# tobifinn/torch-assimilate

Hardware: AMD Instinct MI355X
Metric: local analyses/sec (LETKF, 40-member) (higher is better)
Workload: dtype f32

## Files before the change

### include/mia_letkf.h

```cpp
#ifndef MIA_LETKF_H
#define MIA_LETKF_H

#include <stddef.h>
#include <stdint.h>

#ifdef __cplusplus
extern "C" {
#endif

#define MIA_VERSION 100

#define MIA_OK 0
#define MIA_ERR_NULL (-1)
#define MIA_ERR_SIZE (-2)
#define MIA_ERR_UNSUPPORTED (-3)
#define MIA_ERR_WORKSPACE (-4)
#define MIA_ERR_ALIGN (-5)
#define MIA_ERR_COMM (-6)
#define MIA_ERR_ARG (-7)

#define MIA_FLAG_OVERFLOW 1
#define MIA_FLAG_NOCONV 2
#define MIA_FLAG_NONFINITE 4
#define MIA_FLAG_RETRY 8
// ... 98 lines not shown
                                 int32_t* flags, int32_t* retry_count, void* stream);
int mia_letkf_weights_retry_f32(const float* X, int64_t ldx, int m, int k, int64_t g0, int64_t g1,
                                const float* rec, int64_t P,
                                const int32_t* nbr_cnt, const int32_t* nbr_idx, const double* nbr_w,
                                int p_cap, int p_max, float inf_factor, float gamma,
                                float* Xa, int64_t ldo, int64_t o0, float* W, int32_t* flags, void* stream);
#define MIA_TILE_BOX_OVERFLOW (1 << 30)
#define MIA_STEP_STATUS_SAMPLED 64
#define MIA_STEP_STATUS_NONFINITE 128
int mia_letkf_tile_lists_bytes(int64_t n_points, int p_max, int extra_blocks, size_t* bytes);
int mia_letkf_localize_tiles_f64(int taper, const double* grid_xyz, int64_t g0, int64_t g1,
                                 const double* obs_xyz, int64_t P, int n_coord,
                                 const int32_t* coord_group , const double* gc_c , int n_r,
                                 double gc_eps, int p_max, int extra_blocks, void* tile_lists, size_t tile_lists_bytes,
                                 int32_t* stats, void* ws, size_t ws_bytes, void* stream);
int mia_letkf_localize_tiles_periodic_f64(int taper, const double* grid_xyz, int64_t g0, int64_t g1,
                                          const double* obs_xyz, int64_t P, int n_coord,
                                          const int32_t* coord_group , const double* period ,
                                          const double* gc_c , int n_r, double gc_eps, int p_max, int extra_blocks, void* tile_lists, size_t tile_lists_bytes,
                                          int32_t* stats, void* ws, size_t ws_bytes, void* stream);
int mia_letkf_split_record_bytes(int k, size_t* bytes);
int mia_letkf_pack_split_f32(const float* Yb, const float* d, int k, int64_t P, void* split_rec ,
                             void* stream);
int mia_letkf_analysis_tiles_f32(const float* X, int64_t ldx, int m, int k, int64_t g0, int64_t g1,
                                 const void* split_rec, int64_t P, const void* tile_lists, int p_max, int extra_blocks,
                                 float inf_factor, float* Xa, int64_t ldo, int64_t o0, int32_t* flags,
                                 int32_t* retry_count, void* stream);
int mia_letkf_weights_tiles_f32(const float* X, int64_t ldx, int m, int k, int64_t g0, int64_t g1,
                                const void* split_rec, int64_t P, const void* tile_lists, int p_max, int extra_blocks,
                                float inf_factor, float* Xa, int64_t ldo, int64_t o0, float* W ,
                                int32_t* flags, int32_t* retry_count, void* stream);

int mia_letkf_tiles_cover(int m, int k, int p_max, int extra_blocks, int64_t ldx, int64_t ldo, int64_t n_points, int64_t P,
                          float gamma);
int mia_lketkf_rbf_analysis_tiles_f32(const float* X, int64_t ldx, int m, int k, int64_t g0, int64_t g1,
                                      const float* Yb, const float* d, int64_t P, const void* tile_lists, int p_max,
                                      int extra_blocks, float inf_factor, float gamma, float* Xa, int64_t ldo, int64_t o0,
                                      int32_t* flags, int32_t* retry_count, void* stream);

int mia_letkf_analysis_matfun_fused_f32(const float* X, int64_t ldx, int m, int k, int64_t g0, int64_t g1,
                                        const float* rec, int64_t P,
                                        const double* grid_xyz, int n_coord, const int32_t* coord_group ,
                                        const double* gc_c , int n_r, double gc_eps,
                                        void* index_ws, size_t index_ws_bytes,
                                        int p_max_assumed, float inf_factor, float gamma,
                                        float* Xa, int64_t ldo, int64_t o0, int32_t* flags, int32_t* retry_count,
// ... 274 lines not shown
```

### torch-assimilate_amd/_cabi.py

```python
import ctypes as C
import os

from ._build import LIB_PATH

_lib = None

i32, i64, f32, f64, vp, sz = C.c_int, C.c_int64, C.c_float, C.c_double, C.c_void_p, C.c_size_t


class KernelOp(C.Structure):
    _fields_ = [("op", C.c_int32), ("reserved", C.c_int32), ("value", C.c_double)]


_PROTOS = {
    "mia_version": ([], i32),
    "mia_status_string": ([i32], C.c_char_p),
    "mia_set_option": ([C.c_char_p, i32], i32),
    "mia_get_option": ([C.c_char_p, C.POINTER(C.c_int)], i32),
    "mia_last_analysis_kernel": ([C.c_char_p, i32], i32),
    "mia_last_transform_kernel": ([C.c_char_p, i32], i32),
    "mia_gaspari_cohn_f64": ([vp, i64, vp, vp], i32),
    "mia_gaspari_cohn_f32": ([vp, i64, vp, vp], i32),
    "mia_gaspari_cohn_inf_f64": ([vp, i64, vp, vp], i32),
    "mia_gaspari_cohn_inf_f32": ([vp, i64, vp, vp], i32),
# ... 45 lines not shown
                                      vp, i64, i64, vp, vp, vp, vp], i32),
    "mia_letkf_weights_retry_f64": ([vp, i64, i32, i32, i64, i64, vp, i64, vp, vp, vp, i32, i32, f64, f64,
                                     vp, i64, i64, vp, vp, vp], i32),
    "mia_letkf_weights_f64_cover": ([i32, i32, i64, i64], i32),
    "mia_letkf_weights_matfun_f32": ([vp, i64, i32, i32, i64, i64, vp, i64, vp, vp, vp, i32, i32, f32, f32,
                                      vp, i64, i64, vp, vp, vp, vp], i32),
    "mia_letkf_weights_retry_f32": ([vp, i64, i32, i32, i64, i64, vp, i64, vp, vp, vp, i32, i32, f32, f32,
                                     vp, i64, i64, vp, vp, vp], i32),
    "mia_letkf_index_build_f64": ([vp, i64, i32, C.POINTER(C.c_int32), C.POINTER(f64), i32, vp, sz, vp], i32),
    "mia_letkf_index_build_periodic_f64": ([vp, i64, i32, C.POINTER(C.c_int32), C.POINTER(f64), C.POINTER(f64), i32, vp, sz, vp],
                                           i32),
    "mia_letkf_localize_taper_periodic_f64": ([i32, vp, i64, i64, vp, i64, i32, C.POINTER(C.c_int32), C.POINTER(f64),
                                               C.POINTER(f64), i32, f64, i32, vp, vp, vp, vp, vp, sz, vp], i32),
    "mia_letkf_localize_tiles_periodic_f64": ([i32, vp, i64, i64, vp, i64, i32, C.POINTER(C.c_int32), C.POINTER(f64),
                                               C.POINTER(f64), i32, f64, i32, i32, vp, sz, vp, vp, sz, vp], i32),
    "mia_letkf_analysis_matfun_fused_f32": ([vp, i64, i32, i32, i64, i64, vp, i64, vp, i32, C.POINTER(C.c_int32),
                                             C.POINTER(f64), i32, f64, vp, sz, i32, f32, f32, vp, i64, i64, vp, vp, vp,
                                             vp], i32),
    "mia_letkf_tile_lists_bytes": ([i64, i32, i32, C.POINTER(sz)], i32),
    "mia_letkf_localize_tiles_f64": ([i32, vp, i64, i64, vp, i64, i32, C.POINTER(C.c_int32), C.POINTER(f64), i32, f64,
                                      i32, i32, vp, sz, vp, vp, sz, vp], i32),
    "mia_letkf_split_record_bytes": ([i32, C.POINTER(sz)], i32),
    "mia_letkf_pack_split_f32": ([vp, vp, i32, i64, vp, vp], i32),
    "mia_letkf_analysis_tiles_f32": ([vp, i64, i32, i32, i64, i64, vp, i64, vp, i32, i32, f32, vp, i64, i64, vp, vp, vp], i32),
    "mia_letkf_tiles_cover": ([i32, i32, i32, i32, i64, i64, i64, i64, f32], i32),
    "mia_lketkf_rbf_analysis_tiles_f32": ([vp, i64, i32, i32, i64, i64, vp, vp, i64, vp, i32, i32, f32, f32, vp, i64, i64,
                                           vp, vp, vp], i32),
    "mia_letkf_weights_tiles_f32": ([vp, i64, i32, i32, i64, i64, vp, i64, vp, i32, i32, f32, vp, i64, i64, vp, vp, vp, vp], i32),
    "mia_letkf_analysis_retry_f32": ([vp, i64, i32, i32, i64, i64, vp, i64, vp, vp, vp, i32, i32, f32, f32,
                                      vp, i64, i64, vp, vp], i32),
    "mia_lketkf_rbf_analysis_f32": ([vp, i64, i32, i32, i64, i64, vp, vp, i64, vp, vp, vp, i32, i32, f32, f32,
                                     vp, i64, i64, vp, vp, vp, sz, vp], i32),
    "mia_lketkf_rbf_analysis_f64": ([vp, i64, i32, i32, i64, i64, vp, vp, i64, vp, vp, vp, i32, i32, f64, f64,
                                     vp, i64, i64, vp, vp, vp, sz, vp], i32),
    "mia_etkf_workspace_bytes": ([i32, i64, i32, C.POINTER(sz)], i32),
    "mia_etkf_weights_f32": ([vp, vp, i32, i64, f32, vp, vp, vp, sz, vp], i32),
    "mia_etkf_weights_f64": ([vp, vp, i32, i64, f64, vp, vp, vp, sz, vp], i32),
    "mia_ketkf_workspace_bytes": ([i32, i64, i32, C.POINTER(sz)], i32),
    "mia_ketkf_weights_f32": ([vp, vp, i32, i64, f32, C.POINTER(KernelOp), i32, vp, vp, vp, sz, vp], i32),
    "mia_ketkf_weights_f64": ([vp, vp, i32, i64, f64, C.POINTER(KernelOp), i32, vp, vp, vp, sz, vp], i32),
    "mia_apply_weights_f32": ([vp, i64, i32, i32, i64, i64, vp, vp, i64, i64, vp], i32),
    "mia_apply_weights_f64": ([vp, i64, i32, i32, i64, i64, vp, vp, i64, i64, vp], i32),
    "mia_apply_f64_cover": ([i32, i32, i64, i64, i64], i32),
    "mia_apply_local_f64_cover": ([i32, i32, i64, i64, i64], i32),
    "mia_apply_local_weights_f32": ([vp, i64, i32, i32, i64, i64, vp, vp, i64, i64, vp], i32),
    "mia_apply_local_weights_f64": ([vp, i64, i32, i32, i64, i64, vp, vp, i64, i64, vp], i32),
# ... 153 lines not shown
```

### torch-assimilate_amd/csrc/localize.hip

```cpp
#include <cstdlib>
#include "mia_common.h"
#include "mia_options.h"
#include "mia_localize_dev.h"
#include "mia_pack_dev.h"
#include "mia_tiles.h"

namespace mia {


struct IndexParams {
  const double* obs;
  int64_t P;
  int nc;
  double cutoff[MIA_MAX_COORD];
  int cell_cap;
  IndexHeader* hdr;
  int* start;
  int* cursor;
  int* sorted;
  int* cell_of;
  int* rank_of;
  double* sxyz;
  unsigned nb_bbox;
  PackJob pack;
// ... 530 lines not shown
  unsigned nb_pack = 0;
  if (pack && pack->rec) {
    if ((P + 63) / 64 > 2000000000LL) return MIA_ERR_UNSUPPORTED;
    ip.pack = *pack;
    nb_pack = (unsigned)((P + 63) / 64);
  }
  const size_t pack_lds = nb_pack ? (size_t)64 * (ip.pack.kp + 1) * sizeof(float) : 0;
  index_bbox_dims_kernel<<<dim3(ip.nb_bbox + nb_pack), dim3(kPrepThreads), pack_lds, stream>>>(ip);
  MIA_LAUNCH_CHECK();
  count_k<<<dim3(nbP), dim3(kPrepThreads), 0, stream>>>(ip);
  MIA_LAUNCH_CHECK();
  index_scan_kernel<<<dim3(1), dim3(64), 0, stream>>>(ip);
  MIA_LAUNCH_CHECK();
  ip.scatter_xyz = sort_cells ? 0 : 1;
  scatter_k<<<dim3(nbP), dim3(kPrepThreads), 0, stream>>>(ip);
  MIA_LAUNCH_CHECK();
  if (!sort_cells) return MIA_OK;
  const size_t sort_blocks = L.cap < 8192 ? (L.cap ? L.cap : 1) : 8192;
  sortcell_k<<<dim3((unsigned)sort_blocks), dim3(kPrepThreads), 0, stream>>>(ip);
  MIA_LAUNCH_CHECK();
  return MIA_OK;
}

template <bool PER>
__global__ __launch_bounds__(64) void index_bucket_kernel(IndexParams p) {
  MIA_PREP_PRIORITY();
  MIA_PREP_PRIORITY();
  extern __shared__ __attribute__((aligned(16))) float bk_lds[];
  const bool packs = p.spack.rec != nullptr;
  if (packs) pack_split_lean_request(p.spack, p.P, (int64_t)blockIdx.x, bk_lds);
  const int64_t stride = (int64_t)gridDim.x * blockDim.x;
  for (int q = 0; q < 3; ++q)
    for (int64_t i = blockIdx.x * (int64_t)blockDim.x + threadIdx.x; i < p.zero.n[q]; i += stride) p.zero.ptr[q][i] = 0;
  const int64_t j = blockIdx.x * (int64_t)blockDim.x + threadIdx.x;
  if (j < p.P) {
    IndexHeader* h = p.hdr;
    const bool grid_ok = h->magic == kIndexMagic;
    bool ok = grid_ok && h->bucket_cap > 0;
    for (int c = 0; c < p.nc; ++c) ok = ok && h->cutoff[c] == p.cutoff[c];
    if constexpr (PER)
      for (int c = 0; c < p.nc; ++c) ok = ok && h->period[c] == p.period[c];
    const int cap = h->bucket_cap;
    int id = 0;
    bool skip = false;
    double x[MIA_MAX_COORD] = {0.0, 0.0, 0.0};
    for (int c = 0; c < p.nc; ++c) {
      x[c] = p.obs[j * p.nc + c];
      double f;
      if (PER && p.period[c] > 0.0) {
        x[c] = wrap_coord(x[c], p.period[c]);
        f = floor(x[c] * h->invh[c]);
        f = f > double(h->n[c] - 1) ? double(h->n[c] - 1) : f;
      } else {
        f = floor((x[c] - h->mn[c]) * h->invh[c]);
      }
      if (!(x[c] == x[c])) { skip = true; continue; }
      if (!(f >= 0.0 && f < double(h->n[c]))) { ok = false; continue; }
      id = id * h->n[c] + int(f);
    }
    if (!ok) {
      atomicOr(&h->err, (grid_ok && cap == 0) ? kIndexErrFull : kIndexErrBox);
    } else if (!skip) {
      const int pos = atomicAdd(&p.cursor[id], 1);
      if (pos >= cap) {
        atomicOr(&h->err, kIndexErrFull);
      } else {
        const int64_t e = (int64_t)id * cap + pos;
        p.bidx[e] = int(j);
        for (int c = 0; c < p.nc; ++c) p.bxyz[e * p.nc + c] = x[c];
      }
    }
  }
  if (packs) pack_split_lean_finish(p.spack, p.P, (int64_t)blockIdx.x, bk_lds);
}

int index_bucket_build_impl(const double* obs_xyz, int64_t P, int n_coord, const int32_t* coord_group, const double* gc_c, int n_r,
                            void* ws, size_t ws_bytes, hipStream_t stream, const ZeroJob* zero, bool fresh_box,
                            const SplitPackJob* spack, int* counts, const double* period) {
  if (P <= 0 || n_coord < 1 || n_coord > MIA_MAX_COORD || n_r < 1 || n_r > MIA_MAX_RADII) return MIA_ERR_SIZE;
  if (P > 500000000LL) return MIA_ERR_UNSUPPORTED;
  if (!coord_group || !gc_c || !obs_xyz || !ws) return MIA_ERR_NULL;
  const IndexLayout L = index_layout(ws, P, n_coord);
  if (ws_bytes < L.bytes) return MIA_ERR_WORKSPACE;
  IndexParams ip;
  for (int c = 0; c < MIA_MAX_COORD; ++c) ip.period[c] = (period && c < n_coord) ? period[c] : 0.0;
  ip.periodic = period ? 1 : 0;
  void (*bucket_k)(IndexParams) = period ? index_bucket_kernel<true> : index_bucket_kernel<false>;
  ip.obs = obs_xyz; ip.P = P; ip.nc = n_coord; ip.cell_cap = (int)L.cap;
  for (int c = 0; c < MIA_MAX_COORD; ++c) ip.cutoff[c] = c < n_coord ? 2.0 * gc_c[coord_group[c]] : 1.0;
  ip.hdr = L.hdr; ip.start = L.start; ip.cursor = L.cursor; ip.sorted = L.sorted; ip.cell_of = L.cell_of; ip.rank_of = L.rank_of;
  ip.sxyz = L.sxyz;
  ip.bucket_total = (long long)L.bucket_total; ip.bidx = L.bidx; ip.bxyz = L.bxyz;
  if (counts) ip.cursor = counts;
  ip.pack = PackJob{nullptr, nullptr, nullptr, 0, 0};
  ip.zero = ZeroJob{{nullptr, nullptr, nullptr}, {0, 0, 0}};
  ip.scatter_xyz = 0;
// ... 158 lines not shown
  if (P < 0 || n_coord < 1 || n_coord > MIA_MAX_COORD) return MIA_ERR_SIZE;
  if (P > 2000000000LL) return MIA_ERR_UNSUPPORTED;
  *bytes = index_layout(nullptr, P, n_coord).bytes;
  return MIA_OK;
}

extern "C" int mia_letkf_index_build_f64(const double* obs_xyz, int64_t P, int n_coord, const int32_t* coord_group,
                                         const double* gc_c, int n_r, void* ws, size_t ws_bytes, void* stream) {
  (void)hipGetLastError();
  return index_build_impl(obs_xyz, P, n_coord, coord_group, gc_c, n_r, ws, ws_bytes, (hipStream_t)stream);
}

extern "C" int mia_letkf_index_build_periodic_f64(const double* obs_xyz, int64_t P, int n_coord, const int32_t* coord_group,
                                                  const double* period, const double* gc_c, int n_r, void* ws, size_t ws_bytes,
                                                  void* stream) {
  (void)hipGetLastError();
  if (!period) return MIA_ERR_NULL;
  if (n_coord < 1 || n_coord > MIA_MAX_COORD) return MIA_ERR_SIZE;
  if (check_period(period, n_coord, &period) != MIA_OK) return MIA_ERR_ARG;
  return index_build_impl(obs_xyz, P, n_coord, coord_group, gc_c, n_r, ws, ws_bytes, (hipStream_t)stream, nullptr, nullptr, false,
                          true, period);
}

extern "C" int mia_letkf_localize_f64(const double* grid_xyz, int64_t g0, int64_t g1,
                                      const double* obs_xyz, int64_t P, int n_coord,
                                      const int32_t* coord_group, const double* gc_c, int n_r,
                                      double gc_eps, int p_cap, int32_t* nbr_cnt, int32_t* nbr_idx,
                                      double* nbr_w, int32_t* stats, void* ws, size_t ws_bytes,
                                      void* stream) {
  (void)hipGetLastError();
  return mia::localize_impl(grid_xyz, g0, g1, obs_xyz, P, n_coord, coord_group, gc_c, n_r, gc_eps, p_cap, nbr_cnt,
                            nbr_idx, nbr_w, stats, ws, ws_bytes, (hipStream_t)stream, nullptr, false, nullptr);
}

extern "C" int mia_letkf_localize_taper_f64(int taper, const double* grid_xyz, int64_t g0, int64_t g1,
                                            const double* obs_xyz, int64_t P, int n_coord,
                                            const int32_t* coord_group, const double* gc_c, int n_r,
                                            double gc_eps, int p_cap, int32_t* nbr_cnt, int32_t* nbr_idx,
                                            double* nbr_w, int32_t* stats, void* ws, size_t ws_bytes,
                                            void* stream) {
  (void)hipGetLastError();
  if (taper != MIA_TAPER_GC && taper != MIA_TAPER_GC_INF) return MIA_ERR_SIZE;
  return mia::localize_impl(grid_xyz, g0, g1, obs_xyz, P, n_coord, coord_group, gc_c, n_r, gc_eps, p_cap, nbr_cnt,
                            nbr_idx, nbr_w, stats, ws, ws_bytes, (hipStream_t)stream, nullptr, false, nullptr, taper);
}

// ... 48 lines not shown
```

### torch-assimilate_amd/csrc/mia_tiles.h

```cpp
#pragma once
#include "mia_common.h"

namespace mia {

constexpr int kTileSlack = 8;

static inline int tile_ut_for(int p_max) {
  const int ut = (p_max + kTileSlack + 15) >> 4;
  return ut < 1 ? 1 : ut;
}

struct TileListLayout { size_t hdr, idx, D, bytes; int ut; int64_t ntile; };
static inline TileListLayout tile_list_layout(int64_t ng, int ut) {
  TileListLayout L;
  L.ut = ut;
  L.ntile = (ng + 15) >> 4;
  size_t o = 0;
  L.hdr = o; o = align_up(o + (size_t)(L.ntile > 0 ? L.ntile : 1) * 16, 256);
  L.idx = o; o = align_up(o + (size_t)(L.ntile > 0 ? L.ntile : 1) * 16 * ut * sizeof(int32_t), 256);
  L.D = o; o = align_up(o + (size_t)(L.ntile > 0 ? L.ntile : 1) * ut * 1024, 256);
  L.bytes = o;
  return L;
}

// ... 15 lines not shown
using u4w = __attribute__((ext_vector_type(4))) unsigned;

__device__ __forceinline__ void split8(const float (&x)[8], h8v& hi, h8v& lo) {
  u4w hu, lu;
#pragma unroll
  for (int i = 0; i < 4; ++i) {
    const f2w v = {x[2 * i], x[2 * i + 1]};
    const h2v a = __builtin_convertvector(v, h2v);
    hu[i] = __builtin_bit_cast(unsigned, a);
  }
  asm("s_nop 2\n\t"
      "v_fma_mixlo_f16 %0, %4, -1.0, %8 op_sel:[0,0,0] op_sel_hi:[1,0,0]\n\t"
      "v_fma_mixhi_f16 %0, %4, -1.0, %9 op_sel:[1,0,0] op_sel_hi:[1,0,0]\n\t"
      "v_fma_mixlo_f16 %1, %5, -1.0, %10 op_sel:[0,0,0] op_sel_hi:[1,0,0]\n\t"
      "v_fma_mixhi_f16 %1, %5, -1.0, %11 op_sel:[1,0,0] op_sel_hi:[1,0,0]\n\t"
      "v_fma_mixlo_f16 %2, %6, -1.0, %12 op_sel:[0,0,0] op_sel_hi:[1,0,0]\n\t"
      "v_fma_mixhi_f16 %2, %6, -1.0, %13 op_sel:[1,0,0] op_sel_hi:[1,0,0]\n\t"
      "v_fma_mixlo_f16 %3, %7, -1.0, %14 op_sel:[0,0,0] op_sel_hi:[1,0,0]\n\t"
      "v_fma_mixhi_f16 %3, %7, -1.0, %15 op_sel:[1,0,0] op_sel_hi:[1,0,0]\n\t"
      "s_nop 1"
      : "=&v"(lu[0]), "=&v"(lu[1]), "=&v"(lu[2]), "=&v"(lu[3])
      : "v"(hu[0]), "v"(hu[1]), "v"(hu[2]), "v"(hu[3]), "v"(x[0]), "v"(x[1]), "v"(x[2]), "v"(x[3]), "v"(x[4]), "v"(x[5]),
        "v"(x[6]), "v"(x[7]));
  hi = __builtin_bit_cast(h8v, hu);
  lo = __builtin_bit_cast(h8v, lu);
}
__device__ __forceinline__ void split8_tied(const float (&x)[8], h8v& hi, h8v& lo) {
  u4w hu, lu;
#pragma unroll
  for (int i = 0; i < 4; ++i) {
    const f2w v = {x[2 * i], x[2 * i + 1]};
    const h2v a = __builtin_convertvector(v, h2v);
    hu[i] = __builtin_bit_cast(unsigned, a);
    lu[i] = hu[i];
  }
  asm("v_fma_mixlo_f16 %0, %0, -1.0, %4 op_sel:[0,0,0] op_sel_hi:[1,0,0]\n\t"
      "v_fma_mixhi_f16 %0, %0, -1.0, %5 op_sel:[1,0,0] op_sel_hi:[1,0,0]\n\t"
      "v_fma_mixlo_f16 %1, %1, -1.0, %6 op_sel:[0,0,0] op_sel_hi:[1,0,0]\n\t"
      "v_fma_mixhi_f16 %1, %1, -1.0, %7 op_sel:[1,0,0] op_sel_hi:[1,0,0]\n\t"
      "v_fma_mixlo_f16 %2, %2, -1.0, %8 op_sel:[0,0,0] op_sel_hi:[1,0,0]\n\t"
      "v_fma_mixhi_f16 %2, %2, -1.0, %9 op_sel:[1,0,0] op_sel_hi:[1,0,0]\n\t"
      "v_fma_mixlo_f16 %3, %3, -1.0, %10 op_sel:[0,0,0] op_sel_hi:[1,0,0]\n\t"
      "v_fma_mixhi_f16 %3, %3, -1.0, %11 op_sel:[1,0,0] op_sel_hi:[1,0,0]\n\t"
      "s_nop 1"
      : "+v"(lu[0]), "+v"(lu[1]), "+v"(lu[2]), "+v"(lu[3])
      : "v"(x[0]), "v"(x[1]), "v"(x[2]), "v"(x[3]), "v"(x[4]), "v"(x[5]), "v"(x[6]), "v"(x[7]));
// ... 173 lines not shown
  }
  do { asm volatile("s_waitcnt lgkmcnt(0)" ::: "memory"); __builtin_amdgcn_wave_barrier(); } while (0);
  const int nvalid = P + 1 - j0 < 64 ? (int)(P + 1 - j0) : 64;
  const int nq = nvalid * nc8;
  int r = lane / nc8, c = lane - r * nc8;
  const int dr = 64 / nc8, dc = 64 - dr * nc8;
  for (int q = lane; q < nq; q += 64) {
    const float s = scl[r];
    float x[8];
#pragma unroll
    for (int i = 0; i < 8; ++i) x[i] = 8 * c + i < k ? lds[r * ls + 8 * c + i] * s : 0.0f;
    h8v hi, lo;
    split8(x, hi, lo);
    unsigned char* o = J.rec + (j0 + r) * rb + 32 * c;
    *reinterpret_cast<h8v*>(o) = hi;
    *reinterpret_cast<h8v*>(o + 16) = lo;
    r += dr; c += dc;
    if (c >= nc8) { c -= nc8; ++r; }
  }
}

static inline size_t split_pack_lds(int k) { return ((size_t)64 * ((k + 1) | 1) + 64) * sizeof(float); }

__device__ __forceinline__ void pack_split_lean_request(const SplitPackJob& J, int64_t P, int64_t block, float* lds) {
  const int lane = threadIdx.x & 63;
  const int64_t j = block * 64 + lane;
  const int64_t jc = j < P ? j : (P > 0 ? P - 1 : 0);
  if (P > 0)
    for (int i = 0; i < J.k; ++i)
      __builtin_amdgcn_global_load_lds(reinterpret_cast<const unsigned*>(J.Yb + (int64_t)i * P + jc),
                                       (__attribute__((address_space(3))) void*)(lds + i * 64), 4, 0, 0);
}
__device__ __forceinline__ void pack_split_lean_finish(const SplitPackJob& J, int64_t P, int64_t block, const float* lds) {
  const int lane = threadIdx.x & 63;
  const int k = J.k, nc8 = (k + 7) >> 3, rb = 32 * nc8 + 16;
  const int64_t j = block * 64 + lane;
  const bool real = j < P;
  const float dj = (real && P > 0) ? J.d[j] : 0.0f;
  asm volatile("s_waitcnt vmcnt(0)" ::: "memory");
  __builtin_amdgcn_wave_barrier();
  unsigned mx = 0u;
  if (real)
    for (int i = 0; i < k; ++i) {
      const unsigned a = __float_as_uint(lds[i * 64 + lane]) & 0x7fffffffu;
      mx = a > mx ? a : mx;
    }
  int es;
  const float sc = pow2_scale(mx, 9, &es);
  const float wd = dj * sc;
  const bool bad = mx >= 0x7f800000u || !(fabsf(wd) < 3.0e38f);
  if (j > P) return;
  unsigned char* o = J.rec + j * rb;
  const float E = bad ? __builtin_nanf("") : __uint_as_float((unsigned)(127 - es) << 23);
  *reinterpret_cast<f4w*>(o + 32 * nc8) = f4w{wd, E, 0.0f, 0.0f};
  for (int c = 0; c < nc8; ++c) {
    float x[8];
#pragma unroll
    for (int i = 0; i < 8; ++i) x[i] = (real && 8 * c + i < k) ? lds[(8 * c + i) * 64 + lane] * sc : 0.0f;
    h8v hi, lo;
    split8(x, hi, lo);
    *reinterpret_cast<h8v*>(o + 32 * c) = hi;
    *reinterpret_cast<h8v*>(o + 32 * c + 16) = lo;
  }
}
static inline size_t split_pack_lean_lds(int k) { return (size_t)64 * k * sizeof(float); }

struct ScanParams;
int split_pack_launch(const float* Yb, const float* d, int k, int64_t P, void* rec, hipStream_t stream);
int tile_lists_launch(const double* grid_xyz, int64_t g0, int64_t ng, int64_t P, int n_coord, const int32_t* coord_group,
                      const double* gc_c, int n_r, double gc_eps, int taper, int ut, void* tile_lists, int32_t* stats,
                      void* index_ws, hipStream_t stream, const SplitPackJob* pack, bool bucket = false, const int* counts = nullptr,
                      const double* period = nullptr);
struct Tile2Params {
  const float* X; int64_t ldx; int m, k;
  int64_t g0, ng;
  const unsigned char* rec; int rb, nc8; int64_t zero_rec;
  const int4* thdr; const int32_t* tidx; const f4w* tD;
  float inv_reg, f0, inv_k, cs_phi, cs_psi;
  float* Xa; int64_t ldo, o0; int32_t* flags; int32_t* retry_count;
  int dmax;
  const int2* tab_hdr; const float2* tab_c;
  int seg_len; int64_t seg_stride;
  int* clr_counts; const int* clr_n; unsigned* clr_err; int32_t* err_out;
  int stagger;
};
struct Tile2Housekeeping { int* counts; const int* n; unsigned* err; int32_t* err_out; };
bool tile2_covers(int m, int k, int p_max, int extra_blocks, int64_t ldx, int64_t ldo, int64_t ng);
bool tile2_records_addressable(int k, int64_t P);
// ... 18 lines not shown
```

### torch-assimilate_amd/engine.py

```python
from __future__ import annotations

import ctypes as C
import warnings
from dataclasses import dataclass
from typing import Optional, Sequence

import torch

from . import _cabi

__all__ = ["LetkfEngine", "NeighbourLists", "ObsIndex"]


def _ptr(t: Optional[torch.Tensor]):
    return None if t is None else C.c_void_p(t.data_ptr())


MIA_FLAG_NOCONV = 2


def _read_solve_flags(flags: torch.Tensor) -> int:
    return int(flags[0].item())


# ... 187 lines not shown
        ws = self._workspace("loc", nbytes.value)
        tb = C.c_size_t(0)
        _cabi.check(self.lib.mia_letkf_tile_lists_bytes(g1 - g0, int(p_max), int(extra_blocks), C.byref(tb)),
                    "mia_letkf_tile_lists_bytes")
        lists = torch.empty(max(tb.value, 256), dtype=torch.uint8, device=self.device)
        stats = torch.zeros(2, dtype=torch.int32, device=self.device)
        per = _period_arg(_periods(period, nc), nc)
        _cabi.check(self.lib.mia_letkf_localize_tiles_periodic_f64(
            int(taper), _ptr(grid), g0, g1, _ptr(obs), P, nc, cg, per, rc, len(radii), float(eps), int(p_max),
            int(extra_blocks), _ptr(lists), lists.numel(), _ptr(stats), _ptr(ws), ws.numel(), self._stream()),
            "mia_letkf_localize_tiles_periodic_f64")
        return TileLists(lists, int(p_max), g0, g1, stats, int(extra_blocks))

    def pack_split(self, Yb: torch.Tensor, d: torch.Tensor) -> torch.Tensor:
        Yb = Yb.to(device=self.device, dtype=torch.float32).contiguous()
        d = d.to(device=self.device, dtype=torch.float32).contiguous().reshape(-1)
        k, P = Yb.shape
        rb = C.c_size_t(0)
        _cabi.check(self.lib.mia_letkf_split_record_bytes(k, C.byref(rb)), "mia_letkf_split_record_bytes")
        rec = torch.empty(((P + 1) * rb.value,), dtype=torch.uint8, device=self.device)
        _cabi.check(self.lib.mia_letkf_pack_split_f32(_ptr(Yb), _ptr(d), k, P, _ptr(rec), self._stream()),
                    "mia_letkf_pack_split_f32")
        return rec

    def analysis_tiles(self, X: torch.Tensor, split_rec: torch.Tensor, P: int, tiles: "TileLists", inf_factor: float = 1.0,
                       out: Optional[torch.Tensor] = None):
        X = X.to(device=self.device, dtype=torch.float32).contiguous()
        m, k, G = X.shape
        n = tiles.g1 - tiles.g0
        xa = out if out is not None else torch.empty((m, k, n), dtype=torch.float32, device=self.device)
        flags = torch.zeros(max(n, 1), dtype=torch.int32, device=self.device)
        retry = torch.zeros(1, dtype=torch.int32, device=self.device)
        _cabi.check(self.lib.mia_letkf_analysis_tiles_f32(
            _ptr(X), G, m, k, tiles.g0, tiles.g1, _ptr(split_rec), int(P), _ptr(tiles.lists), tiles.p_max, tiles.extra_blocks,
            float(inf_factor), _ptr(xa), xa.shape[-1], 0, _ptr(flags), _ptr(retry), self._stream()),
            "mia_letkf_analysis_tiles_f32")
        return xa, flags[:n], retry

    def analysis_tiles_rbf(self, X: torch.Tensor, Yb: torch.Tensor, d: torch.Tensor, tiles: "TileLists", inf_factor: float,
                           rbf_gamma: float, out: Optional[torch.Tensor] = None):
        X = X.to(device=self.device, dtype=torch.float32).contiguous()
        Yb = Yb.to(device=self.device, dtype=torch.float32).contiguous()
        d = d.to(device=self.device, dtype=torch.float32).contiguous().reshape(-1)
        m, k, G = X.shape
        n = tiles.g1 - tiles.g0
        xa = out if out is not None else torch.empty((m, k, n), dtype=torch.float32, device=self.device)
# ... 665 lines not shown
```

Measured before the change: 2.579 billion.

## Overlap bucket-index loads with split packing via manual vmcnt ladder and rotated LDS layout

Restructures the fused bucket-index/split-pack kernel. It issues the header, coordinate and d loads up front and reads the header with wave readlanes. Hand-written vmcnt wait ladders let the bucket atomic overlap the Yb-to-LDS loads and chunk stores. Packing is rebalanced so each lane handles (row, chunk) quads over a rotated LDS layout that avoids bank conflicts, and zeroing moves to the end. It also adds a standalone bucket_pack entry point, at the cost of fragile inline assembly and a large branch ladder.

After: 2.700 billion, median of 6. 1.05x the previous value.

```diff
diff --git a/include/mia_letkf.h b/include/mia_letkf.h
--- a/include/mia_letkf.h
+++ b/include/mia_letkf.h
@@ -144,6 +144,10 @@
 int mia_letkf_split_record_bytes(int k, size_t* bytes);
 int mia_letkf_pack_split_f32(const float* Yb, const float* d, int k, int64_t P, void* split_rec ,
                              void* stream);
+int mia_letkf_bucket_pack_f32(const double* obs_xyz, int64_t P, int n_coord, const int32_t* coord_group ,
+                              const double* gc_c , int n_r, const double* period , void* ws,
+                              size_t ws_bytes, const float* Yb, const float* d, int k, void* split_rec ,
+                              void* stream);
 int mia_letkf_analysis_tiles_f32(const float* X, int64_t ldx, int m, int k, int64_t g0, int64_t g1,
                                  const void* split_rec, int64_t P, const void* tile_lists, int p_max, int extra_blocks,
                                  float inf_factor, float* Xa, int64_t ldo, int64_t o0, int32_t* flags,
diff --git a/torch-assimilate_amd/_cabi.py b/torch-assimilate_amd/_cabi.py
--- a/torch-assimilate_amd/_cabi.py
+++ b/torch-assimilate_amd/_cabi.py
@@ -91,6 +91,8 @@
                                       i32, i32, vp, sz, vp, vp, sz, vp], i32),
     "mia_letkf_split_record_bytes": ([i32, C.POINTER(sz)], i32),
     "mia_letkf_pack_split_f32": ([vp, vp, i32, i64, vp, vp], i32),
+    "mia_letkf_bucket_pack_f32": ([vp, i64, i32, C.POINTER(C.c_int32), C.POINTER(f64), i32, C.POINTER(f64), vp, sz,
+                                   vp, vp, i32, vp, vp], i32),
     "mia_letkf_analysis_tiles_f32": ([vp, i64, i32, i32, i64, i64, vp, i64, vp, i32, i32, f32, vp, i64, i64, vp, vp, vp], i32),
     "mia_letkf_tiles_cover": ([i32, i32, i32, i32, i64, i64, i64, i64, f32], i32),
     "mia_lketkf_rbf_analysis_tiles_f32": ([vp, i64, i32, i32, i64, i64, vp, vp, i64, vp, i32, i32, f32, f32, vp, i64, i64,
diff --git a/torch-assimilate_amd/csrc/localize.hip b/torch-assimilate_amd/csrc/localize.hip
--- a/torch-assimilate_amd/csrc/localize.hip
+++ b/torch-assimilate_amd/csrc/localize.hip
@@ -576,56 +576,139 @@
   return MIA_OK;
 }
 
+__device__ __forceinline__ unsigned bk_request_u32(const void* p) {
+  unsigned v;
+  asm volatile("global_load_dword %0, %1, off" : "=v"(v) : "v"(p) : "memory");
+  return v;
+}
+__device__ __forceinline__ double bk_request_f64(const double* p) {
+  double v;
+  asm volatile("global_load_dwordx2 %0, %1, off" : "=v"(v) : "v"(p) : "memory");
+  return v;
+}
+__device__ __forceinline__ unsigned bk_hdr_u32(unsigned hw, size_t byte_off) {
+  return (unsigned)__builtin_amdgcn_readlane((int)hw, (int)(byte_off / 4));
+}
+__device__ __forceinline__ double bk_hdr_f64(unsigned hw, size_t byte_off) {
+  return __hiloint2double(__builtin_amdgcn_readlane((int)hw, (int)(byte_off / 4) + 1), __builtin_amdgcn_readlane((int)hw, (int)(byte_off / 4)));
+}
+#define MIA_BK_HDR_U32(hw, field) bk_hdr_u32(hw, offsetof(IndexHeader, field))
+#define MIA_BK_HDR_F64(hw, field, c) bk_hdr_f64(hw, offsetof(IndexHeader, field) + 8 * (size_t)(c))
+#define MIA_BK_HDR_I32(hw, field, c) (int)bk_hdr_u32(hw, offsetof(IndexHeader, field) + 4 * (size_t)(c))
+#define MIA_BK_WAIT_STEP(OP, N) "s_cmp_eq_u32 %" #OP ", " #N "\n\ts_cbranch_scc1 .Lbk_w" #N "_%=\n\t"
+#define MIA_BK_WAIT_ARM(N) ".Lbk_w" #N "_%=:\n\ts_waitcnt vmcnt(" #N ")\n\ts_branch .Lbk_end_%=\n"
+#define MIA_BK_WAIT_LADDER(OP) \
+  MIA_BK_WAIT_STEP(OP, 0) MIA_BK_WAIT_STEP(OP, 1) MIA_BK_WAIT_STEP(OP, 2) MIA_BK_WAIT_STEP(OP, 3) MIA_BK_WAIT_STEP(OP, 4) MIA_BK_WAIT_STEP(OP, 5) MIA_BK_WAIT_STEP(OP, 6) \
+  MIA_BK_WAIT_STEP(OP, 7) MIA_BK_WAIT_STEP(OP, 8) MIA_BK_WAIT_STEP(OP, 9) MIA_BK_WAIT_STEP(OP, 10) MIA_BK_WAIT_STEP(OP, 11) MIA_BK_WAIT_STEP(OP, 12) MIA_BK_WAIT_STEP(OP, 13) \
+  MIA_BK_WAIT_STEP(OP, 14) MIA_BK_WAIT_STEP(OP, 15) MIA_BK_WAIT_STEP(OP, 16) MIA_BK_WAIT_STEP(OP, 17) MIA_BK_WAIT_STEP(OP, 18) MIA_BK_WAIT_STEP(OP, 19) MIA_BK_WAIT_STEP(OP, 20) \
+  MIA_BK_WAIT_STEP(OP, 21) MIA_BK_WAIT_STEP(OP, 22) MIA_BK_WAIT_STEP(OP, 23) MIA_BK_WAIT_STEP(OP, 24) MIA_BK_WAIT_STEP(OP, 25) MIA_BK_WAIT_STEP(OP, 26) MIA_BK_WAIT_STEP(OP, 27) \
+  MIA_BK_WAIT_STEP(OP, 28) MIA_BK_WAIT_STEP(OP, 29) MIA_BK_WAIT_STEP(OP, 30) MIA_BK_WAIT_STEP(OP, 31) MIA_BK_WAIT_STEP(OP, 32) MIA_BK_WAIT_STEP(OP, 33) MIA_BK_WAIT_STEP(OP, 34) \
+  MIA_BK_WAIT_STEP(OP, 35) MIA_BK_WAIT_STEP(OP, 36) MIA_BK_WAIT_STEP(OP, 37) MIA_BK_WAIT_STEP(OP, 38) MIA_BK_WAIT_STEP(OP, 39) MIA_BK_WAIT_STEP(OP, 40) MIA_BK_WAIT_STEP(OP, 41) \
+  MIA_BK_WAIT_STEP(OP, 42) MIA_BK_WAIT_STEP(OP, 43) MIA_BK_WAIT_STEP(OP, 44) MIA_BK_WAIT_STEP(OP, 45) MIA_BK_WAIT_STEP(OP, 46) MIA_BK_WAIT_STEP(OP, 47) MIA_BK_WAIT_STEP(OP, 48) \
+  MIA_BK_WAIT_STEP(OP, 49) MIA_BK_WAIT_STEP(OP, 50) MIA_BK_WAIT_STEP(OP, 51) MIA_BK_WAIT_STEP(OP, 52) MIA_BK_WAIT_STEP(OP, 53) MIA_BK_WAIT_STEP(OP, 54) MIA_BK_WAIT_STEP(OP, 55) \
+  MIA_BK_WAIT_STEP(OP, 56) MIA_BK_WAIT_STEP(OP, 57) MIA_BK_WAIT_STEP(OP, 58) MIA_BK_WAIT_STEP(OP, 59) MIA_BK_WAIT_STEP(OP, 60) MIA_BK_WAIT_STEP(OP, 61) MIA_BK_WAIT_STEP(OP, 62) \
+  "s_waitcnt vmcnt(63)\n\ts_branch .Lbk_end_%=\n" \
+  MIA_BK_WAIT_ARM(0) MIA_BK_WAIT_ARM(1) MIA_BK_WAIT_ARM(2) MIA_BK_WAIT_ARM(3) MIA_BK_WAIT_ARM(4) MIA_BK_WAIT_ARM(5) MIA_BK_WAIT_ARM(6) \
+  MIA_BK_WAIT_ARM(7) MIA_BK_WAIT_ARM(8) MIA_BK_WAIT_ARM(9) MIA_BK_WAIT_ARM(10) MIA_BK_WAIT_ARM(11) MIA_BK_WAIT_ARM(12) MIA_BK_WAIT_ARM(13) \
+  MIA_BK_WAIT_ARM(14) MIA_BK_WAIT_ARM(15) MIA_BK_WAIT_ARM(16) MIA_BK_WAIT_ARM(17) MIA_BK_WAIT_ARM(18) MIA_BK_WAIT_ARM(19) MIA_BK_WAIT_ARM(20) \
+  MIA_BK_WAIT_ARM(21) MIA_BK_WAIT_ARM(22) MIA_BK_WAIT_ARM(23) MIA_BK_WAIT_ARM(24) MIA_BK_WAIT_ARM(25) MIA_BK_WAIT_ARM(26) MIA_BK_WAIT_ARM(27) \
+  MIA_BK_WAIT_ARM(28) MIA_BK_WAIT_ARM(29) MIA_BK_WAIT_ARM(30) MIA_BK_WAIT_ARM(31) MIA_BK_WAIT_ARM(32) MIA_BK_WAIT_ARM(33) MIA_BK_WAIT_ARM(34) \
+  MIA_BK_WAIT_ARM(35) MIA_BK_WAIT_ARM(36) MIA_BK_WAIT_ARM(37) MIA_BK_WAIT_ARM(38) MIA_BK_WAIT_ARM(39) MIA_BK_WAIT_ARM(40) MIA_BK_WAIT_ARM(41) \
+  MIA_BK_WAIT_ARM(42) MIA_BK_WAIT_ARM(43) MIA_BK_WAIT_ARM(44) MIA_BK_WAIT_ARM(45) MIA_BK_WAIT_ARM(46) MIA_BK_WAIT_ARM(47) MIA_BK_WAIT_ARM(48) \
+  MIA_BK_WAIT_ARM(49) MIA_BK_WAIT_ARM(50) MIA_BK_WAIT_ARM(51) MIA_BK_WAIT_ARM(52) MIA_BK_WAIT_ARM(53) MIA_BK_WAIT_ARM(54) MIA_BK_WAIT_ARM(55) \
+  MIA_BK_WAIT_ARM(56) MIA_BK_WAIT_ARM(57) MIA_BK_WAIT_ARM(58) MIA_BK_WAIT_ARM(59) MIA_BK_WAIT_ARM(60) MIA_BK_WAIT_ARM(61) MIA_BK_WAIT_ARM(62) \
+  ".Lbk_end_%=:"
+#define MIA_BK_WAIT_FIRST(hw, x0, x1, x2, dbits, rows) \
+  asm volatile(MIA_BK_WAIT_LADDER(5) : "+v"(hw), "+v"(x0), "+v"(x1), "+v"(x2), "+v"(dbits) : "s"(rows) : "scc", "memory")
+#define MIA_BK_WAIT_ATOMIC(pos, stores) asm volatile(MIA_BK_WAIT_LADDER(1) : "+v"(pos) : "s"(stores) : "scc", "memory")
+
 template <bool PER>
 __global__ __launch_bounds__(64) void index_bucket_kernel(IndexParams p) {
   MIA_PREP_PRIORITY();
   MIA_PREP_PRIORITY();
   extern __shared__ __attribute__((aligned(16))) float bk_lds[];
   const bool packs = p.spack.rec != nullptr;
-  if (packs) pack_split_lean_request(p.spack, p.P, (int64_t)blockIdx.x, bk_lds);
-  const int64_t stride = (int64_t)gridDim.x * blockDim.x;
-  for (int q = 0; q < 3; ++q)
-    for (int64_t i = blockIdx.x * (int64_t)blockDim.x + threadIdx.x; i < p.zero.n[q]; i += stride) p.zero.ptr[q][i] = 0;
-  const int64_t j = blockIdx.x * (int64_t)blockDim.x + threadIdx.x;
+  const int lane = threadIdx.x;
+  const int64_t j0 = blockIdx.x * (int64_t)blockDim.x;
+  const int64_t j = j0 + lane;
+  const int64_t jc = j < p.P ? j : p.P - 1;
+  unsigned hw = bk_request_u32(reinterpret_cast<const unsigned*>(p.hdr) + lane);
+  double x[MIA_MAX_COORD];
+#pragma unroll
+  for (int c = 0; c < MIA_MAX_COORD; ++c) x[c] = bk_request_f64(p.obs + jc * p.nc + (c < p.nc ? c : 0));
+  unsigned dbits = bk_request_u32(packs ? static_cast<const void*>(p.spack.d + jc) : static_cast<const void*>(p.hdr));
+  int rows = 0;
+  if (packs) {
+    pack_split_lean_request(p.spack, p.P, j0, bk_lds);
+    rows = p.spack.k;
+  }
+  MIA_BK_WAIT_FIRST(hw, x[0], x[1], x[2], dbits, rows);
+  const bool grid_ok = MIA_BK_HDR_U32(hw, magic) == kIndexMagic;
+  const int cap = (int)MIA_BK_HDR_U32(hw, bucket_cap);
+  bool ok = grid_ok && cap > 0;
+  int id = 0;
+  bool skip = false;
+#pragma unroll
+  for (int c = 0; c < MIA_MAX_COORD; ++c) {
+    if (c >= p.nc) continue;
+    ok = ok && MIA_BK_HDR_F64(hw, cutoff, c) == p.cutoff[c];
+    if constexpr (PER) ok = ok && MIA_BK_HDR_F64(hw, period, c) == p.period[c];
+    const int n_c = MIA_BK_HDR_I32(hw, n, c);
+    const double invh_c = MIA_BK_HDR_F64(hw, invh, c);
+    double f;
+    if (PER && p.period[c] > 0.0) {
+      x[c] = wrap_coord(x[c], p.period[c]);
+      f = floor(x[c] * invh_c);
+      f = f > double(n_c - 1) ? double(n_c - 1) : f;
+    } else {
+      f = floor((x[c] - MIA_BK_HDR_F64(hw, mn, c)) * invh_c);
+    }
+    if (!(x[c] == x[c])) { skip = true; continue; }
+    if (!(f >= 0.0 && f < double(n_c))) { ok = false; continue; }
+    id = id * n_c + int(f);
+  }
+  const bool bins = j < p.P && ok && !skip;
+  int pos = bins ? 1 : 0;
+  {
+    const int* slot = p.cursor + (bins ? id : lane);
+    asm volatile("global_atomic_add %0, %1, %0, off sc0" : "+v"(pos) : "v"(slot) : "memory");
+  }
+  int stores = 0;
+  float sc = 1.0f, E = 1.0f;
+  if (packs) {
+    const int nc8 = (p.spack.k + 7) >> 3;
+    const int nvalid = p.P + 1 - j0 < 64 ? (int)(p.P + 1 - j0) : 64;
+    stores = 2 * ((nvalid * nc8 + 63) >> 6);
+    asm volatile("s_waitcnt vmcnt(1)" ::: "memory");
+    __builtin_amdgcn_wave_barrier();
+    if ((p.spack.k & 7) == 0) {
+      sc = pack_split_lean_scale<false>(p.spack, p.P, j, __uint_as_float(dbits), bk_lds, E);
+      pack_split_lean_chunks<false>(p.spack, p.P, j0, sc, bk_lds);
+    } else {
+      sc = pack_split_lean_scale<true>(p.spack, p.P, j, __uint_as_float(dbits), bk_lds, E);
+      pack_split_lean_chunks<true>(p.spack, p.P, j0, sc, bk_lds);
+    }
+  }
+  MIA_BK_WAIT_ATOMIC(pos, stores);
   if (j < p.P) {
-    IndexHeader* h = p.hdr;
-    const bool grid_ok = h->magic == kIndexMagic;
-    bool ok = grid_ok && h->bucket_cap > 0;
-    for (int c = 0; c < p.nc; ++c) ok = ok && h->cutoff[c] == p.cutoff[c];
-    if constexpr (PER)
-      for (int c = 0; c < p.nc; ++c) ok = ok && h->period[c] == p.period[c];
-    const int cap = h->bucket_cap;
-    int id = 0;
-    bool skip = false;
-    double x[MIA_MAX_COORD] = {0.0, 0.0, 0.0};
-    for (int c = 0; c < p.nc; ++c) {
-      x[c] = p.obs[j * p.nc + c];
-      double f;
-      if (PER && p.period[c] > 0.0) {
-        x[c] = wrap_coord(x[c], p.period[c]);
-        f = floor(x[c] * h->invh[c]);
-        f = f > double(h->n[c] - 1) ? double(h->n[c] - 1) : f;
-      } else {
-        f = floor((x[c] - h->mn[c]) * h->invh[c]);
-      }
-      if (!(x[c] == x[c])) { skip = true; continue; }
-      if (!(f >= 0.0 && f < double(h->n[c]))) { ok = false; continue; }
-      id = id * h->n[c] + int(f);
-    }
     if (!ok) {
-      atomicOr(&h->err, (grid_ok && cap == 0) ? kIndexErrFull : kIndexErrBox);
+      atomicOr(&p.hdr->err, (grid_ok && cap == 0) ? kIndexErrFull : kIndexErrBox);
     } else if (!skip) {
-      const int pos = atomicAdd(&p.cursor[id], 1);
       if (pos >= cap) {
-        atomicOr(&h->err, kIndexErrFull);
+        atomicOr(&p.hdr->err, kIndexErrFull);
       } else {
         const int64_t e = (int64_t)id * cap + pos;
         p.bidx[e] = int(j);
-        for (int c = 0; c < p.nc; ++c) p.bxyz[e * p.nc + c] = x[c];
+#pragma unroll
+        for (int c = 0; c < MIA_MAX_COORD; ++c)
+          if (c < p.nc) p.bxyz[e * p.nc + c] = x[c];
       }
     }
   }
-  if (packs) pack_split_lean_finish(p.spack, p.P, (int64_t)blockIdx.x, bk_lds);
+  if (packs) pack_split_lean_tail(p.spack, p.P, j, __uint_as_float(dbits), sc, E);
+  const int64_t stride = (int64_t)gridDim.x * blockDim.x;
+  for (int q = 0; q < 3; ++q)
+    for (int64_t i = j; i < p.zero.n[q]; i += stride) p.zero.ptr[q][i] = 0;
 }
 
 int index_bucket_build_impl(const double* obs_xyz, int64_t P, int n_coord, const int32_t* coord_group, const double* gc_c, int n_r,
@@ -830,6 +913,21 @@
                           true, period);
 }
 
+extern "C" int mia_letkf_bucket_pack_f32(const double* obs_xyz, int64_t P, int n_coord, const int32_t* coord_group,
+                                         const double* gc_c, int n_r, const double* period, void* ws, size_t ws_bytes,
+                                         const float* Yb, const float* d, int k, void* rec, void* stream) {
+  (void)hipGetLastError();
+  if (P < 1 || k < 1 || n_coord < 1 || n_coord > MIA_MAX_COORD || n_r < 1 || n_r > MIA_MAX_RADII) return MIA_ERR_SIZE;
+  if (!coord_group || !gc_c || !obs_xyz || !ws || !Yb || !d || !rec) return MIA_ERR_NULL;
+  for (int c = 0; c < n_coord; ++c) if (coord_group[c] < 0 || coord_group[c] >= n_r) return MIA_ERR_SIZE;
+  for (int r = 0; r < n_r; ++r) if (!(gc_c[r] > 0.0)) return MIA_ERR_SIZE;
+  if ((((uintptr_t)ws) & 255) || (((uintptr_t)rec) & 15)) return MIA_ERR_ALIGN;
+  if (check_period(period, n_coord, &period) != MIA_OK) return MIA_ERR_ARG;
+  const SplitPackJob sj{Yb, d, (unsigned char*)rec, k};
+  return index_bucket_build_impl(obs_xyz, P, n_coord, coord_group, gc_c, n_r, ws, ws_bytes, (hipStream_t)stream, nullptr, true, &sj,
+                                 nullptr, period);
+}
+
 extern "C" int mia_letkf_localize_f64(const double* grid_xyz, int64_t g0, int64_t g1,
                                       const double* obs_xyz, int64_t P, int n_coord,
                                       const int32_t* coord_group, const double* gc_c, int n_r,
diff --git a/torch-assimilate_amd/csrc/mia_tiles.h b/torch-assimilate_amd/csrc/mia_tiles.h
--- a/torch-assimilate_amd/csrc/mia_tiles.h
+++ b/torch-assimilate_amd/csrc/mia_tiles.h
@@ -61,6 +61,28 @@
       : "=&v"(lu[0]), "=&v"(lu[1]), "=&v"(lu[2]), "=&v"(lu[3])
       : "v"(hu[0]), "v"(hu[1]), "v"(hu[2]), "v"(hu[3]), "v"(x[0]), "v"(x[1]), "v"(x[2]), "v"(x[3]), "v"(x[4]), "v"(x[5]),
         "v"(x[6]), "v"(x[7]));
+  hi = __builtin_bit_cast(h8v, hu);
+  lo = __builtin_bit_cast(h8v, lu);
+}
+__device__ __forceinline__ void split8_inplace(float (&x)[8], h8v& hi, h8v& lo) {
+  u4w hu, lu;
+#pragma unroll
+  for (int i = 0; i < 4; ++i) {
+    const f2w v = {x[2 * i], x[2 * i + 1]};
+    const h2v a = __builtin_convertvector(v, h2v);
+    hu[i] = __builtin_bit_cast(unsigned, a);
+    lu[i] = __float_as_uint(x[2 * i]);
+  }
+  asm("v_fma_mixlo_f16 %0, %4, -1.0, %0 op_sel:[0,0,0] op_sel_hi:[1,0,0]\n\t"
+      "v_fma_mixhi_f16 %0, %4, -1.0, %8 op_sel:[1,0,0] op_sel_hi:[1,0,0]\n\t"
+      "v_fma_mixlo_f16 %1, %5, -1.0, %1 op_sel:[0,0,0] op_sel_hi:[1,0,0]\n\t"
+      "v_fma_mixhi_f16 %1, %5, -1.0, %9 op_sel:[1,0,0] op_sel_hi:[1,0,0]\n\t"
+      "v_fma_mixlo_f16 %2, %6, -1.0, %2 op_sel:[0,0,0] op_sel_hi:[1,0,0]\n\t"
+      "v_fma_mixhi_f16 %2, %6, -1.0, %10 op_sel:[1,0,0] op_sel_hi:[1,0,0]\n\t"
+      "v_fma_mixlo_f16 %3, %7, -1.0, %3 op_sel:[0,0,0] op_sel_hi:[1,0,0]\n\t"
+      "v_fma_mixhi_f16 %3, %7, -1.0, %11 op_sel:[1,0,0] op_sel_hi:[1,0,0]"
+      : "+v"(lu[0]), "+v"(lu[1]), "+v"(lu[2]), "+v"(lu[3])
+      : "v"(hu[0]), "v"(hu[1]), "v"(hu[2]), "v"(hu[3]), "v"(x[1]), "v"(x[3]), "v"(x[5]), "v"(x[7]));
   hi = __builtin_bit_cast(h8v, hu);
   lo = __builtin_bit_cast(h8v, lu);
 }
@@ -280,48 +302,74 @@
 
 static inline size_t split_pack_lds(int k) { return ((size_t)64 * ((k + 1) | 1) + 64) * sizeof(float); }
 
-__device__ __forceinline__ void pack_split_lean_request(const SplitPackJob& J, int64_t P, int64_t block, float* lds) {
+constexpr int kLeanRot = 16;
+__device__ __forceinline__ void pack_split_lean_request(const SplitPackJob& J, int64_t P, int64_t j0, float* lds) {
   const int lane = threadIdx.x & 63;
-  const int64_t j = block * 64 + lane;
-  const int64_t jc = j < P ? j : (P > 0 ? P - 1 : 0);
-  if (P > 0)
-    for (int i = 0; i < J.k; ++i)
-      __builtin_amdgcn_global_load_lds(reinterpret_cast<const unsigned*>(J.Yb + (int64_t)i * P + jc),
-                                       (__attribute__((address_space(3))) void*)(lds + i * 64), 4, 0, 0);
-}
-__device__ __forceinline__ void pack_split_lean_finish(const SplitPackJob& J, int64_t P, int64_t block, const float* lds) {
+  for (int i = 0; i < J.k; ++i) {
+    const int64_t j = j0 + ((lane + kLeanRot * (i >> 3)) & 63);
+    const int64_t jc = j < P ? j : P - 1;
+    __builtin_amdgcn_global_load_lds(reinterpret_cast<const unsigned*>(J.Yb + (int64_t)i * P + jc),
+                                     (__attribute__((address_space(3))) void*)(lds + i * 64), 4, 0, 0);
+  }
+}
+template <bool RAGGED>
+__device__ __forceinline__ float pack_split_lean_scale(const SplitPackJob& J, int64_t P, int64_t j, float dj, const float* lds, float& E) {
   const int lane = threadIdx.x & 63;
   const int k = J.k, nc8 = (k + 7) >> 3, rb = 32 * nc8 + 16;
-  const int64_t j = block * 64 + lane;
   const bool real = j < P;
-  const float dj = (real && P > 0) ? J.d[j] : 0.0f;
-  asm volatile("s_waitcnt vmcnt(0)" ::: "memory");
-  __builtin_amdgcn_wave_barrier();
   unsigned mx = 0u;
-  if (real)
-    for (int i = 0; i < k; ++i) {
-      const unsigned a = __float_as_uint(lds[i * 64 + lane]) & 0x7fffffffu;
-      mx = a > mx ? a : mx;
-    }
+#pragma nounroll
+  for (int i0 = 0; i0 < k; i0 += 8) {
+    const float* w = lds + i0 * 64 + ((lane - kLeanRot * (i0 >> 3)) & 63);
+    unsigned a[8];
+#pragma unroll
+    for (int u = 0; u < 8; ++u) a[u] = __float_as_uint(w[64 * u]) & 0x7fffffffu;
+#pragma unroll
+    for (int u = 0; u < 8; ++u) mx = (a[u] > mx && (!RAGGED || i0 + u < k)) ? a[u] : mx;
+  }
+  mx = real ? mx : 0u;
   int es;
   const float sc = pow2_scale(mx, 9, &es);
-  const float wd = dj * sc;
-  const bool bad = mx >= 0x7f800000u || !(fabsf(wd) < 3.0e38f);
-  if (j > P) return;
-  unsigned char* o = J.rec + j * rb;
-  const float E = bad ? __builtin_nanf("") : __uint_as_float((unsigned)(127 - es) << 23);
-  *reinterpret_cast<f4w*>(o + 32 * nc8) = f4w{wd, E, 0.0f, 0.0f};
-  for (int c = 0; c < nc8; ++c) {
-    float x[8];
-#pragma unroll
-    for (int i = 0; i < 8; ++i) x[i] = (real && 8 * c + i < k) ? lds[(8 * c + i) * 64 + lane] * sc : 0.0f;
-    h8v hi, lo;
-    split8(x, hi, lo);
-    *reinterpret_cast<h8v*>(o + 32 * c) = hi;
-    *reinterpret_cast<h8v*>(o + 32 * c + 16) = lo;
-  }
-}
-static inline size_t split_pack_lean_lds(int k) { return (size_t)64 * k * sizeof(float); }
+  const bool bad = mx >= 0x7f800000u || !(fabsf((real ? dj : 0.0f) * sc) < 3.0e38f);
+  E = bad ? __builtin_nanf("") : __uint_as_float((unsigned)(127 - es) << 23);
+  return sc;
+}
+__device__ __forceinline__ void pack_split_lean_tail(const SplitPackJob& J, int64_t P, int64_t j, float dj, float sc, float E) {
+  const int nc8 = (J.k + 7) >> 3, rb = 32 * nc8 + 16;
+  if (j <= P) *reinterpret_cast<f4w*>(J.rec + j * rb + 32 * nc8) = f4w{(j < P ? dj : 0.0f) * sc, E, 0.0f, 0.0f};
+}
+template <bool RAGGED>
+__device__ __forceinline__ void pack_split_lean_chunks(const SplitPackJob& J, int64_t P, int64_t j0, float sc, const float* lds) {
+  const int lane = threadIdx.x & 63;
+  const int k = J.k, nc8 = (k + 7) >> 3, rb = 32 * nc8 + 16;
+  const int nvalid = P + 1 - j0 < 64 ? (int)(P + 1 - j0) : 64;
+  const int nreal = P - j0 < 64 ? (int)(P - j0) : 64;
+  const int nq = nvalid * nc8;
+  unsigned char* rec0 = J.rec + (uint64_t)blockIdx.x * (uint64_t)(unsigned)(64 * rb);
+  const unsigned inv = nc8 > 1 ? 0xffffffffu / (unsigned)nc8 + 1u : 0u;
+#pragma nounroll
+  for (int q0 = 0; q0 < nq; q0 += 64) {
+    int q = lane;
+    asm volatile("" : "+v"(q));
+    q += q0;
+    const int r = nc8 > 1 ? (int)__umulhi((unsigned)q, inv) : q, c = q - r * nc8;
+    const float s = __shfl(sc, r & 63, 64);
+    if (q < nq) {
+      const float* w = lds + 8 * c * 64 + ((r - kLeanRot * c) & 63);
+      float x[8];
+#pragma unroll
+      for (int i = 0; i < 8; ++i) x[i] = w[64 * i];
+#pragma unroll
+      for (int i = 0; i < 8; ++i) x[i] = (r < nreal && (!RAGGED || 8 * c + i < k)) ? x[i] * s : 0.0f;
+      h8v hi, lo;
+      split8_inplace(x, hi, lo);
+      const unsigned o = (unsigned)(r * rb + 32 * c);
+      *reinterpret_cast<h8v*>(rec0 + o) = hi;
+      *reinterpret_cast<h8v*>(rec0 + o + 16) = lo;
+    }
+  }
+}
+static inline size_t split_pack_lean_lds(int k) { return (size_t)64 * 8 * ((k + 7) >> 3) * sizeof(float); }
 
 struct ScanParams;
 int split_pack_launch(const float* Yb, const float* d, int k, int64_t P, void* rec, hipStream_t stream);
diff --git a/torch-assimilate_amd/engine.py b/torch-assimilate_amd/engine.py
--- a/torch-assimilate_amd/engine.py
+++ b/torch-assimilate_amd/engine.py
@@ -233,6 +233,33 @@
         _cabi.check(self.lib.mia_letkf_pack_split_f32(_ptr(Yb), _ptr(d), k, P, _ptr(rec), self._stream()),
                     "mia_letkf_pack_split_f32")
         return rec
+
+    def bucket_pack(self, obs_xyz, radii: Sequence[float], Yb: torch.Tensor, d: torch.Tensor,
+                    coord_group: Optional[Sequence[int]] = None, period=None, ws: Optional[torch.Tensor] = None):
+        obs = self._dev(obs_xyz, torch.float64)
+        if obs.dim() == 1:
+            obs = obs[:, None].contiguous()
+        Yb = Yb.to(device=self.device, dtype=torch.float32).contiguous()
+        d = d.to(device=self.device, dtype=torch.float32).contiguous().reshape(-1)
+        k, P = Yb.shape
+        nc = obs.shape[1]
+        if obs.shape[0] != P or d.numel() != P:
+            raise ValueError("obs_xyz, Yb and d disagree on the number of observations")
+        radii = [float(r) for r in (radii if hasattr(radii, "__len__") else [radii])]
+        coord_group = [0] * nc if coord_group is None else [int(c) for c in coord_group]
+        if ws is None:
+            nbytes = C.c_size_t(0)
+            _cabi.check(self.lib.mia_letkf_localize_workspace_bytes(P, nc, C.byref(nbytes)), "localize_workspace_bytes")
+            ws = torch.empty(max(nbytes.value, 256), dtype=torch.uint8, device=self.device)
+        rb = C.c_size_t(0)
+        _cabi.check(self.lib.mia_letkf_split_record_bytes(k, C.byref(rb)), "mia_letkf_split_record_bytes")
+        rec = torch.empty(((P + 1) * rb.value,), dtype=torch.uint8, device=self.device)
+        cg = (C.c_int32 * nc)(*coord_group)
+        rc = (C.c_double * len(radii))(*radii)
+        _cabi.check(self.lib.mia_letkf_bucket_pack_f32(_ptr(obs), P, nc, cg, rc, len(radii), _periods(period, nc), _ptr(ws),
+                                                       ws.numel(), _ptr(Yb), _ptr(d), k, _ptr(rec), self._stream()),
+                    "mia_letkf_bucket_pack_f32")
+        return rec, ws
 
     def analysis_tiles(self, X: torch.Tensor, split_rec: torch.Tensor, P: int, tiles: "TileLists", inf_factor: float = 1.0,
                        out: Optional[torch.Tensor] = None):
```
